# sunnyHelen/JPerceiver

Measured on AMD Instinct MI355X. Metric: train images/sec (full train step, synthetic 3-frame batches), higher is better.
Workload: dtype f32

## Files before the change

### jperceiver_amd/csrc/conv_pack.hip

```cpp
#include "conv_pack.h"
#include "igemm_p9.h"
#include "igemm_p9s.h"
#include "scale.h"
#include <algorithm>

namespace {

struct JpPackJob {
    const float* w;
    float* wp;
    long total, begin;
    int mode, p[6];
};
static_assert(sizeof(JpPackJob) == 64, "JpPackJob layout");
__host__ __device__ inline int jp_cdiv_d(int a, int b) { return (a + b - 1) / b; }

__device__ __forceinline__ float pack_slot_sum(const float* wc, int pl) {
    const int a = pl >> 3, b = (pl >> 2) & 1, r = (pl >> 1) & 1, sx = pl & 1;
    const int y0 = a ? (r ? 2 : 0) : (r ? 1 : 0), y1 = a ? (r ? 2 : 1) : (r ? 2 : 0);
    const int x0 = b ? (sx ? 2 : 0) : (sx ? 1 : 0), x1 = b ? (sx ? 2 : 1) : (sx ? 2 : 0);
    float v = 0.f;
    for (int dy = y0; dy <= y1; ++dy)
        for (int dx = x0; dx <= x1; ++dx) v += wc[dy * 3 + dx];
    return v;
}

__device__ __forceinline__ float pack_elem(int mode, const float* __restrict__ w, long i, const int* p, float sc = 1.f) {
    switch (mode) {
        case PACK_TAP: {
            const int Cout = p[0], Cin = p[1], KHW = p[2], Cp = p[3], for_dgrad = p[4];
            const int rows = for_dgrad ? Cin : Cout, red = for_dgrad ? Cout : Cin;
            const int c = (int)(i % Cp);
            const long t = i / Cp;
            const int r = (int)(t % rows), tap = (int)(t / rows);
            if (c >= red) return 0.f;
            const int co = for_dgrad ? c : r, ci = for_dgrad ? r : c;
            return w[((size_t)co * Cin + ci) * KHW + tap];
        }
        case PACK_ROWMAJOR: {
            const int Cin = p[1], KHW = p[2], CP = p[3], Kp = p[4];
            const int k = (int)(i % Kp), m = (int)(i / Kp);
            const int tap = k / CP, c = k - tap * CP;
            return (tap < KHW && c < Cin) ? w[((size_t)m * Cin + c) * KHW + tap] : 0.f;
        }
        case PACK_SEG: {
            const int Cout = p[0], Cin = p[1], c_off = p[2], C = p[3], Cp = p[4], up = p[5];
            const int c = (int)(i % Cp);
            const long t = i / Cp;
            const int co = (int)(t % Cout), pl = (int)(t / Cout);
            if (c >= C) return 0.f;
            const float* wc = w + ((size_t)co * Cin + c_off + c) * 9;
            return up ? pack_slot_sum(wc, pl) : wc[pl];
        }
        case PACK_UP_DGRAD: {
            const int Cout = p[0], Cin = p[1], c_off = p[2], Cx = p[3], Cp = p[4];
            const int co = (int)(i % Cp);
            const long t = i / Cp;
            const int c = (int)(t % Cx), pl = (int)(t / Cx);
            if (co >= Cout) return 0.f;
            return pack_slot_sum(w + ((size_t)co * Cin + c_off + c) * 9, pl);
        }
        case PACK_FRAG: {
            const int Cout = p[0], Cin = p[1], for_dgrad = p[2], BMT = p[3], KHW = p[4];
            const int rows = for_dgrad ? Cin : Cout, red = for_dgrad ? Cout : Cin;
            const long per_tile = ((long)((red + 31) / 32) * KHW * 4 + P9_QAHEAD + 1) * 8 * BMT;
            const int mt = (int)(i / per_tile);
            long t = i - (long)mt * per_tile;
            const int j = (int)(t & 3); t >>= 2;
            const int m = mt * BMT + (int)(t % BMT);
            t /= BMT;
            const int par = (int)(t & 1); t >>= 1;
            const long step = t * 4 + j;
            const int s_ = (int)(step & 15);
            const long tc = step >> 4;
            const int tap = (int)(tc % KHW);
            const int c = (int)(tc / KHW) * 32 + 2 * s_ + par;
            if (m >= rows || c >= red) return 0.f;
            const int co = for_dgrad ? c : m, ci = for_dgrad ? m : c;
            return w[((size_t)co * Cin + ci) * KHW + tap];
        }
        case PACK_SPLIT: {
            const int Cout = p[0], Cin = p[1], for_dgrad = p[2], BMT = p[3], KHW = p[4], KGS = p[5];
            const int rows = for_dgrad ? Cin : Cout, red = for_dgrad ? Cout : Cin;
            const long nsteps = (long)(red / (16 * KGS)) * KHW * KGS;
            const long per_tile = (nsteps + P9S_AHEAD) * (JP_NS * 8) * BMT;
            const int mt = (int)(i / per_tile);
            long t = i - (long)mt * per_tile;
            const int w4 = (int)(t & 3); t >>= 2;
            const int m = mt * BMT + (int)(t % BMT);
            t /= BMT;
            const int khalf = (int)(t & 1); t >>= 1;
            const int sp = (int)(t % JP_NS);
            const long U = t / JP_NS;
            if (U >= nsteps || m >= rows) return 0.f;
            const int stage = (int)(U / (KHW * KGS)), u = (int)(U % (KHW * KGS));
            const int tap = u / KGS, kg = u % KGS;
            const int c = stage * 16 * KGS + kg * 16 + khalf * 8 + 2 * w4;
            float v[2];
#pragma unroll
            for (int k = 0; k < 2; ++k) {
                const int cc = c + k;
                const int co = for_dgrad ? cc : m, ci = for_dgrad ? m : cc;
                v[k] = cc < red ? w[((size_t)co * Cin + ci) * KHW + tap] : 0.f;
            }
            unsigned sq[3];
            jp_split_ns(v[0], v[1], sc, sq);
            return __uint_as_float(sp == 0 ? sq[0] : (sp == 1 ? sq[1] : sq[2]));
        }
        case PACK_SPLIT7: {
            const int Cout = p[0], Cin = p[1];
            const int w4 = (int)(i & 3), m = (int)((i >> 2) & 63), khalf = (int)((i >> 8) & 1);
            const long t = i >> 9;
            const int sp = (int)(t % JP_NS);
            const long U = t / JP_NS;
            const int c = (int)(U >> 2), ky = 2 * (int)(U & 3) + khalf;
            float v[2];
#pragma unroll
            for (int k = 0; k < 2; ++k) {
                const int kx = 2 * w4 + k;
                v[k] = (c < Cin && m < Cout && ky < 7 && kx < 7) ? w[(((size_t)m * Cin + c) * 7 + ky) * 7 + kx] : 0.f;
            }
            unsigned sq[3];
            jp_split_ns(v[0], v[1], sc, sq);
            return __uint_as_float(sp == 0 ? sq[0] : (sp == 1 ? sq[1] : sq[2]));
        }
        case PACK_SPLITUPD: {
            const int Cout = p[0], Cin = p[1], c_off = p[2], Cx = p[3];
            const long nsteps = (long)((Cout + 31) / 32 * 2) * 16;
            const long per_tile = (nsteps + P9S_AHEAD) * (JP_NS * 1024);
            const int mt = (int)(i / per_tile);
            long t = i - (long)mt * per_tile;
            const int w4 = (int)(t & 3); t >>= 2;
            const int c = mt * 128 + (int)(t & 127); t >>= 7;
            const int khalf = (int)(t & 1); t >>= 1;
            const int sp = (int)(t % JP_NS);
            const long U = t / JP_NS;
            if (U >= nsteps || c >= Cx) return 0.f;
            const int stage = (int)(U >> 4), q = (int)(U & 15);
            const int co = stage * 16 + khalf * 8 + 2 * w4;
            float v[2];
#pragma unroll
            for (int k = 0; k < 2; ++k)
                v[k] = co + k < Cout ? pack_slot_sum(w + ((size_t)(co + k) * Cin + c_off + c) * 9, q) : 0.f;
            unsigned sq[3];
            jp_split_ns(v[0], v[1], sc, sq);
            return __uint_as_float(sp == 0 ? sq[0] : (sp == 1 ? sq[1] : sq[2]));
        }
        case PACK_SPLITSEG: {
            const int Cout = p[0], Cin = p[1], c_off = p[2], C = p[3], up = p[4];
            const int T = up ? 4 : 9, MT = Cout / 128;
            const long tile = (long)((C + 15) / 16) * T * (JP_NS * 1024);
            const int cm = (int)(i / tile);
            if (cm >= (up ? 4 : 1) * MT) return 0.f;
            long t = i - (long)cm * tile;
            const int cls = cm / MT, mt = cm - cls * MT;
            const int w4 = (int)(t & 3); t >>= 2;
            const int row = (int)(t & 127); t >>= 7;
            const int khalf = (int)(t & 1); t >>= 1;
            const int sp = (int)(t % JP_NS);
            const int U = (int)(t / JP_NS);
            const int stage = U / T, tap = U - stage * T;
            const int c = stage * 16 + khalf * 8 + 2 * w4, co = mt * 128 + row;
            float v[2];
#pragma unroll
            for (int k = 0; k < 2; ++k) {
                const float* wc = w + ((size_t)co * Cin + c_off + c + k) * 9;
                v[k] = (c + k < C && co < Cout) ? (up ? pack_slot_sum(wc, cls * 4 + tap) : wc[tap]) : 0.f;
            }
            unsigned sq[3];
            jp_split_ns(v[0], v[1], sc, sq);
            return __uint_as_float(sp == 0 ? sq[0] : (sp == 1 ? sq[1] : sq[2]));
        }
        case PACK_FRAGSEG: {
            const int Cout = p[0], Cin = p[1], c_off = p[2], C = p[3], KP = p[4], up = p[5];
            const int T = up ? 4 : 9, MT = Cout / 128;
            const long tile = (long)((C + 2 * KP - 1) / (2 * KP)) * T * KP / 4 * 1024;
            const int cm = (int)(i / tile);
            long t = i - (long)cm * tile;
            const int cls = cm / MT, mt = cm - cls * MT;
            const int j = (int)(t & 3); t >>= 2;
            const int row = (int)(t & 127); t >>= 7;
            const int par = (int)(t & 1); t >>= 1;
            const long step = t * 4 + j;
            const int stage = (int)(step / (T * KP)), rem = (int)(step - (long)stage * (T * KP));
            const int tap = rem / KP, s_ = rem - tap * KP;
            const int c = stage * 2 * KP + 2 * s_ + par, co = mt * 128 + row;
            if (c >= C || co >= Cout) return 0.f;
            const float* wc = w + ((size_t)co * Cin + c_off + c) * 9;
            return up ? pack_slot_sum(wc, cls * 4 + tap) : wc[tap];
        }
        default: {
            const int Cout = p[0], Cin = p[1], c_off = p[2];
            const int t = (int)(i % 9), co = (int)((i / 9) % Cout), c = (int)(i / (9 * (long)Cout));
            return w[((size_t)co * Cin + c_off + c) * 9 + 8 - t];
        }
    }
}

__device__ __forceinline__ int pack_hdr(int mode) { return (mode == PACK_SPLIT || mode == PACK_SPLITUPD || mode == PACK_SPLIT7) ? JP_PACK_HDR : 0; }
__device__ __forceinline__ float pack_scale_of(const JpPackJob& j) {
    if (!JP_PACK_HDR) return 1.f;
    if (j.mode == PACK_SPLIT || j.mode == PACK_SPLITUPD || j.mode == PACK_SPLIT7) return j.wp[0];
    if (j.mode == PACK_SPLITSEG) return *(j.wp - j.p[5]);
    return 1.f;
}
constexpr int PSL = 32;
__device__ __forceinline__ float* pack_scale_hdr(const JpPackJob& j, long* n) {
    const bool seg = j.mode == PACK_SPLITSEG && j.p[2] == 0;
    const bool upd = j.mode == PACK_SPLITUPD;
    const bool s7 = j.mode == PACK_SPLIT7;
    if (!JP_PACK_HDR || !(j.mode == PACK_SPLIT || seg || upd || s7)) return nullptr;
    *n = (long)j.p[0] * j.p[1] * ((seg || upd) ? 9 : (s7 ? 49 : j.p[4]));
    return seg ? j.wp - j.p[5] : j.wp;
}
__device__ __forceinline__ void pack_scale_zero(const JpPackJob& j) {
    long n;
    float* hdr = pack_scale_hdr(j, &n);
    if (hdr && threadIdx.x == 0) reinterpret_cast<unsigned*>(hdr)[2] = 0u;
}
__device__ __forceinline__ void pack_scale_reduce(const JpPackJob& j, int slice) {
    long n;
    float* hdr = pack_scale_hdr(j, &n);
    if (!hdr) return;
    const long per = (n + PSL - 1) / PSL, beg = slice * per, end = min(n, beg + per);
    unsigned m = 0;
    for (long i = beg + threadIdx.x; i < end; i += 256) m = max(m, jp_amag(__float_as_uint(j.w[i])));
#pragma unroll
    for (int o = 32; o > 0; o >>= 1) m = max(m, (unsigned)__shfl_xor((int)m, o, 64));
    if ((threadIdx.x & 63) == 0 && m) atomicMax(reinterpret_cast<unsigned*>(hdr) + 2, m);
}
__device__ __forceinline__ void pack_scale_finish(const JpPackJob& j) {
    long n;
    float* hdr = pack_scale_hdr(j, &n);
    if (!hdr || threadIdx.x) return;
    const int k = jp_scale_exp(hdr[2] * ((j.mode == PACK_SPLITSEG || j.mode == PACK_SPLITUPD) ? 4.f : 1.f));
    hdr[0] = jp_exp2i(k);
    hdr[1] = jp_exp2i(-k);
    hdr[2] = hdr[3] = 0.f;
}
__global__ __launch_bounds__(64) void pack_scale_zero_one_kernel(JpPackJob job) { pack_scale_zero(job); }
__global__ __launch_bounds__(256) void pack_scale_reduce_one_kernel(JpPackJob job) { pack_scale_reduce(job, blockIdx.x); }
__global__ __launch_bounds__(64) void pack_scale_finish_one_kernel(JpPackJob job) { pack_scale_finish(job); }
__global__ __launch_bounds__(64) void pack_scale_zero_kernel(const JpPackJob* __restrict__ jobs, int njobs) {
    const int q = blockIdx.x * 64 + threadIdx.x;
    if (q < njobs) { long n; float* hdr = pack_scale_hdr(jobs[q], &n); if (hdr) reinterpret_cast<unsigned*>(hdr)[2] = 0u; }
}
__global__ __launch_bounds__(256) void pack_scale_reduce_kernel(const JpPackJob* __restrict__ jobs, int njobs) {
    pack_scale_reduce(jobs[blockIdx.y], blockIdx.x);
}
__global__ __launch_bounds__(64) void pack_scale_finish_kernel(const JpPackJob* __restrict__ jobs, int njobs) {
    const int q = blockIdx.x * 64 + threadIdx.x;
    if (q < njobs) {
        long n;
        float* hdr = pack_scale_hdr(jobs[q], &n);
        if (hdr) {
            const int k = jp_scale_exp(hdr[2] * ((jobs[q].mode == PACK_SPLITSEG || jobs[q].mode == PACK_SPLITUPD) ? 4.f : 1.f));
            hdr[0] = jp_exp2i(k);
            hdr[1] = jp_exp2i(-k);
            hdr[2] = hdr[3] = 0.f;
        }
    }
}

__global__ __launch_bounds__(256) void pack_one_kernel(JpPackJob job) {
    const int hdr = pack_hdr(job.mode);
    const float sc = pack_scale_of(job);
    for (long i = (long)blockIdx.x * 256 + threadIdx.x; i < job.total - hdr; i += (long)gridDim.x * 256)
        job.wp[hdr + i] = pack_elem(job.mode, job.w, i, job.p, sc);
}

__global__ __launch_bounds__(256) void pack_replay_kernel(const JpPackJob* __restrict__ jobs, int njobs, long total) {
    const long groups = (total + 3) >> 2;
    for (long g4 = (long)blockIdx.x * 256 + threadIdx.x; g4 < groups; g4 += (long)gridDim.x * 256) {
        const long g = g4 << 2;
        int lo = 0, hi = njobs - 1;
        while (lo < hi) {
            const int mid = (lo + hi + 1) >> 1;
            if (jobs[mid].begin <= g) lo = mid; else hi = mid - 1;
        }
        const JpPackJob& j = jobs[lo];
        const long i = g - j.begin;
        if (i >= j.total) continue;
        if (j.mode == PACK_SPLIT || j.mode == PACK_SPLITSEG) continue;
        if (j.mode == PACK_FRAG && i + 4 <= j.total) {
            const int* p = j.p;
            const int Cout = p[0], Cin = p[1], for_dgrad = p[2], BMT = p[3], KHW = p[4];
            const int rows = for_dgrad ? Cin : Cout, red = for_dgrad ? Cout : Cin;
            const long per_tile = ((long)((red + 31) / 32) * KHW * 4 + P9_QAHEAD + 1) * 8 * BMT;
            const int mt = (int)(i / per_tile);
            long t = (i - (long)mt * per_tile) >> 2;
            const int m = mt * BMT + (int)(t % BMT);
            t /= BMT;
            const int par = (int)(t & 1); t >>= 1;
            const long step = t * 4;
            const int s0 = (int)(step & 15);
            const long tc = step >> 4;
            const int tap = (int)(tc % KHW), c0 = (int)(tc / KHW) * 32 + 2 * s0 + par;
            float4 v = make_float4(0.f, 0.f, 0.f, 0.f);
            if (m < rows) {
                const size_t cs = for_dgrad ? (size_t)Cin * KHW : (size_t)KHW;
                const float* wb = j.w + (for_dgrad ? (size_t)m * KHW : (size_t)m * Cin * KHW) + tap;
                if (c0 < red) v.x = wb[(size_t)c0 * cs];
                if (c0 + 2 < red) v.y = wb[(size_t)(c0 + 2) * cs];
                if (c0 + 4 < red) v.z = wb[(size_t)(c0 + 4) * cs];
                if (c0 + 6 < red) v.w = wb[(size_t)(c0 + 6) * cs];
            }
            *reinterpret_cast<float4*>(j.wp + i) = v;
        } else {
            const int hdr = pack_hdr(j.mode);
            const float sc = hdr ? pack_scale_of(j) : 1.f;
#pragma unroll
            for (int k = 0; k < 4; ++k)
                if (i + k >= hdr && i + k < j.total) j.wp[i + k] = pack_elem(j.mode, j.w, i + k - hdr, j.p, sc);
        }
    }
}

__device__ __forceinline__ int split_job_items(const JpPackJob& j) {
    const int* p = j.p;
    if (j.mode == PACK_SPLIT) {
        const int rows = p[2] ? p[1] : p[0], red = p[2] ? p[0] : p[1];
        return jp_cdiv_d(rows, p[3]) * (red / (16 * p[5])) * (p[3] / 64);
    }
    if (j.mode == PACK_SPLITSEG) return (p[0] / 128) * ((p[3] + 15) / 16) * 2;
    return 0;
}
__global__ __launch_bounds__(256) void pack_split_replay_kernel(const JpPackJob* __restrict__ jobs, int njobs) {
    __shared__ float tile[64 * 16 * 9 + 64];
    constexpr int MAXJ = 2048;
    __shared__ int pre[MAXJ + 1];
    const int t = threadIdx.x;
    for (int q = t; q < njobs && q < MAXJ; q += 256) pre[q + 1] = split_job_items(jobs[q]);
    if (t == 0) pre[0] = 0;
    __syncthreads();
    if (t == 0)
        for (int q = 1; q <= njobs && q <= MAXJ; ++q) pre[q] += pre[q - 1];
    __syncthreads();
    const int nj = min(njobs, MAXJ), total_items = pre[nj];
    for (int item = blockIdx.x; item < total_items; item += gridDim.x) {
        __syncthreads();
        int lo = 0, hi = nj - 1;
        while (lo < hi) {
            const int mid = (lo + hi + 1) >> 1;
            if (pre[mid] <= item) lo = mid; else hi = mid - 1;
        }
        const int jj = lo, loc = item - pre[lo];
        const JpPackJob& j = jobs[jj];
        const int* p = j.p;
        unsigned* out = reinterpret_cast<unsigned*>(j.wp) + pack_hdr(j.mode);
        if (j.mode == PACK_SPLIT) {
            const float wsc = JP_PACK_HDR ? j.wp[0] : 1.f;
            const int Cout = p[0], Cin = p[1], for_dgrad = p[2], BMT = p[3], KHW = p[4], KGS = p[5];
            const int rows = for_dgrad ? Cin : Cout, red = for_dgrad ? Cout : Cin;
            const int CS = 16 * KGS, nst = red / CS, rch = BMT / 64;
            const int rc = loc % rch, stage = (loc / rch) % nst, mt = loc / (rch * nst);
            const int m0 = mt * BMT + rc * 64, c0 = stage * CS;
            const int RUN = CS * KHW;
            if (!for_dgrad) {
                for (int e = t; e < 64 * RUN; e += 256) {
                    const int r = e / RUN, o = e - r * RUN;
                    tile[e] = (m0 + r < rows) ? j.w[((size_t)(m0 + r) * Cin + c0) * KHW + o] : 0.f;
                }
            } else {
                const int RUNd = 64 * KHW;
                for (int e = t; e < CS * RUNd; e += 256) {
                    const int c = e / RUNd, o = e - c * RUNd;
                    tile[e] = (m0 + o / KHW < rows) ? j.w[((size_t)(c0 + c) * Cin + m0) * KHW + o] : 0.f;
                }
            }
            __syncthreads();
            const long nsteps = (long)nst * KHW * KGS;
            const long per_tile = (nsteps + P9S_AHEAD) * (JP_NS * 8) * BMT;
            const int trip = KHW * KGS * 2 * 64;
            for (int e = t; e < trip; e += 256) {
                const int r = e & 63, kh = (e >> 6) & 1, u = e >> 7;
                const int tap = u / KGS, kg = u - tap * KGS;
                jp_u32x4 w0, w1, w2;
#pragma unroll
                for (int k = 0; k < 4; ++k) {
                    const int c = kg * 16 + kh * 8 + 2 * k;
                    const float a = for_dgrad ? tile[(c * 64 + r) * KHW + tap] : tile[(r * CS + c) * KHW + tap];
                    const float b = for_dgrad ? tile[((c + 1) * 64 + r) * KHW + tap] : tile[(r * CS + c + 1) * KHW + tap];
                    unsigned sq[3];
                    jp_split_ns(a, b, wsc, sq);
                    w0[k] = sq[0]; w1[k] = sq[1]; w2[k] = sq[2];
                }
                const long U = (long)stage * KHW * KGS + u;
                unsigned* q = out + (long)mt * per_tile + ((U * JP_NS) * 2 + kh) * (long)BMT * 4 + (long)(rc * 64 + r) * 4;
                *reinterpret_cast<jp_u32x4*>(q) = w0;
                *reinterpret_cast<jp_u32x4*>(q + 2L * BMT * 4) = w1;
                if (JP_NS == 3) *reinterpret_cast<jp_u32x4*>(q + 4L * BMT * 4) = w2;
            }
        } else {
            const int Cout = p[0], Cin = p[1], c_off = p[2], C = p[3], up = p[4];
            const int T = up ? 4 : 9, MT = Cout / 128, nst = (C + 15) / 16;
            const int rc = loc & 1, stage = (loc >> 1) % nst, mt = (loc >> 1) / nst;
            const int m0 = mt * 128 + rc * 64, c0 = stage * 16;
            for (int e = t; e < 64 * 144; e += 256) {
                const int r = e / 144, o = e - r * 144, c = o / 9;
                tile[e] = (c0 + c < C && m0 + r < Cout) ? j.w[((size_t)(m0 + r) * Cin + c_off + c0) * 9 + o] : 0.f;
            }
            __syncthreads();
            const long tl = (long)nst * T * (JP_NS * 1024);
            const int ncls = up ? 4 : 1, trip = ncls * T * 2 * 64;
            const float wsc = pack_scale_of(j);
            for (int e = t; e < trip; e += 256) {
                const int r = e & 63, kh = (e >> 6) & 1, ct = e >> 7, tap = ct % T, cls = ct / T;
                jp_u32x4 w0, w1, w2;
#pragma unroll
                for (int k = 0; k < 4; ++k) {
                    const int c = kh * 8 + 2 * k;
                    const float* wa = tile + (r * 16 + c) * 9;
                    const float a = up ? pack_slot_sum(wa, cls * 4 + tap) : wa[tap];
                    const float b = up ? pack_slot_sum(wa + 9, cls * 4 + tap) : wa[9 + tap];
                    unsigned sq[3];
                    jp_split_ns(a, b, wsc, sq);
                    w0[k] = sq[0]; w1[k] = sq[1]; w2[k] = sq[2];
                }
                const long U = (long)stage * T + tap;
                unsigned* q = out + (long)(cls * MT + mt) * tl + ((U * JP_NS) * 2 + kh) * 512L + (long)(rc * 64 + r) * 4;
                *reinterpret_cast<jp_u32x4*>(q) = w0;
                *reinterpret_cast<jp_u32x4*>(q + 1024) = w1;
                if (JP_NS == 3) *reinterpret_cast<jp_u32x4*>(q + 2048) = w2;
            }
        }
    }
}

thread_local JpPackJob* g_pack_rec = nullptr;
thread_local int g_pack_rec_n = 0, g_pack_rec_cap = 0;

}

void do_pack(int mode, const float* w, float* wp, long total, int p0, int p1, int p2, int p3, int p4, int p5, hipStream_t st) {
    JpPackJob j{w, wp, total, 0, mode, {p0, p1, p2, p3, p4, p5}};
    if (g_pack_rec) {
        if (g_pack_rec_n < g_pack_rec_cap) g_pack_rec[g_pack_rec_n] = j;
        ++g_pack_rec_n;
    }
    if (JP_PACK_HDR && (mode == PACK_SPLIT || mode == PACK_SPLITUPD || mode == PACK_SPLIT7 || (mode == PACK_SPLITSEG && p2 == 0))) {
        hipLaunchKernelGGL(pack_scale_zero_one_kernel, dim3(1), dim3(64), 0, st, j);
        hipLaunchKernelGGL(pack_scale_reduce_one_kernel, dim3(PSL), dim3(256), 0, st, j);
        hipLaunchKernelGGL(pack_scale_finish_one_kernel, dim3(1), dim3(64), 0, st, j);
    }
    hipLaunchKernelGGL(pack_one_kernel, dim3((int)std::min<long>((total + 255) / 256, 4096)), dim3(256), 0, st, j);
}

void pack_weights(const float* w, float* wp, int Cout, int Cin, int KHW, int Cp, int for_dgrad, hipStream_t st) {
    do_pack(PACK_TAP, w, wp, (long)KHW * (for_dgrad ? Cin : Cout) * Cp, Cout, Cin, KHW, Cp, for_dgrad, 0, st);
}

extern "C" int jp_pack_job_bytes(void) { return (int)sizeof(JpPackJob); }

extern "C" int jp_pack_record_begin(void* host_jobs, int max_jobs) {
    JP_CHECK_ARG(host_jobs && max_jobs > 0 && !g_pack_rec, "pack_record_begin: bad args or a recording is already open");
    g_pack_rec = (JpPackJob*)host_jobs;
    g_pack_rec_n = 0;
    g_pack_rec_cap = max_jobs;
    return JP_OK;
}

extern "C" int jp_pack_record_end(void) {
    g_pack_rec = nullptr;
    return g_pack_rec_n;
}

extern "C" int jp_pack_mode_is_split(int mode) { return (mode == PACK_SPLIT || mode == PACK_SPLITSEG) ? 1 : 0; }
extern "C" int jp_pack_replay(const void* jobs, int njobs, long total_elems, long generic_elems, void* stream) {
    JP_CHECK_ARG(jobs && njobs > 0 && total_elems > 0, "pack_replay: bad args");
    const long gen = (generic_elems > 0 && generic_elems < total_elems) ? generic_elems : total_elems;
    if (JP_PACK_HDR)
    {
        hipLaunchKernelGGL(pack_scale_zero_kernel, dim3((njobs + 63) / 64), dim3(64), 0, (hipStream_t)stream, (const JpPackJob*)jobs, njobs);
        hipLaunchKernelGGL(pack_scale_reduce_kernel, dim3(PSL, njobs), dim3(256), 0, (hipStream_t)stream, (const JpPackJob*)jobs, njobs);
        hipLaunchKernelGGL(pack_scale_finish_kernel, dim3((njobs + 63) / 64), dim3(64), 0, (hipStream_t)stream, (const JpPackJob*)jobs, njobs);
    }
    hipLaunchKernelGGL(pack_replay_kernel, dim3((int)std::min<long>((gen + 4095) / 4096, 16384)), dim3(256), 0,
                       (hipStream_t)stream, (const JpPackJob*)jobs, njobs, gen);
    for (int off = 0; off < njobs; off += 2048)
        hipLaunchKernelGGL(pack_split_replay_kernel, dim3(4096), dim3(256), 0, (hipStream_t)stream, (const JpPackJob*)jobs + off,
                           std::min(2048, njobs - off));
    JP_LAUNCH_CHECK();
}
```

Measured before the change: 126.7.

## Add fast weight-pack replay path with vectorized reduce, walk scheduling, pipelined split pack

Adds an env-gated fast path, on by default, for weight-pack replay. The scale reduction now reads float4 vectors. The generic replay kernel gives each block a contiguous range, walks jobs linearly instead of binary-searching per element, and gets a vectorized PACK_TAP case. A new persistent split-pack kernel stages coalesced tiles through registers and shared memory, prefetching the next item while the current one is stored. This targets per-step weight repacking overhead, at the cost of more code and register pressure.

After: 123.9. -2.2%, worse.

```diff
diff --git a/jperceiver_amd/csrc/conv_pack.hip b/jperceiver_amd/csrc/conv_pack.hip
--- a/jperceiver_amd/csrc/conv_pack.hip
+++ b/jperceiver_amd/csrc/conv_pack.hip
@@ -248,6 +248,30 @@
 __global__ __launch_bounds__(256) void pack_scale_reduce_kernel(const JpPackJob* __restrict__ jobs, int njobs) {
     pack_scale_reduce(jobs[blockIdx.y], blockIdx.x);
 }
+__global__ __launch_bounds__(256) void pack_scale_reduce4_kernel(const JpPackJob* __restrict__ jobs, int njobs) {
+    const JpPackJob& j = jobs[blockIdx.y];
+    long n;
+    float* hdr = pack_scale_hdr(j, &n);
+    if (!hdr) return;
+    const int t = threadIdx.x, slice = blockIdx.x;
+    const long head = min(n, (long)((16 - ((uintptr_t)j.w & 15)) & 15) >> 2);
+    const float4* w4 = reinterpret_cast<const float4*>(j.w + head);
+    const long n4 = (n - head) >> 2, per = (n4 + PSL - 1) / PSL, beg = slice * per, end = min(n4, beg + per);
+    unsigned m = 0;
+    for (long i = beg + t; i < end; i += 256) {
+        const float4 v = w4[i];
+        m = max(max(m, jp_amag(__float_as_uint(v.x))), jp_amag(__float_as_uint(v.y)));
+        m = max(max(m, jp_amag(__float_as_uint(v.z))), jp_amag(__float_as_uint(v.w)));
+    }
+    if (slice == 0) {
+        if (t < head) m = max(m, jp_amag(__float_as_uint(j.w[t])));
+        const long tail = head + (n4 << 2);
+        if (tail + t < n) m = max(m, jp_amag(__float_as_uint(j.w[tail + t])));
+    }
+#pragma unroll
+    for (int o = 32; o > 0; o >>= 1) m = max(m, (unsigned)__shfl_xor((int)m, o, 64));
+    if ((t & 63) == 0 && m) atomicMax(reinterpret_cast<unsigned*>(hdr) + 2, m);
+}
 __global__ __launch_bounds__(64) void pack_scale_finish_kernel(const JpPackJob* __restrict__ jobs, int njobs) {
     const int q = blockIdx.x * 64 + threadIdx.x;
     if (q < njobs) {
@@ -269,6 +293,57 @@
         job.wp[hdr + i] = pack_elem(job.mode, job.w, i, job.p, sc);
 }
 
+template <bool FAST>
+__device__ __forceinline__ void pack_replay_group(const JpPackJob& j, long i) {
+    if (i >= j.total) return;
+    if (j.mode == PACK_SPLIT || j.mode == PACK_SPLITSEG) return;
+    if (j.mode == PACK_FRAG && i + 4 <= j.total) {
+        const int* p = j.p;
+        const int Cout = p[0], Cin = p[1], for_dgrad = p[2], BMT = p[3], KHW = p[4];
+        const int rows = for_dgrad ? Cin : Cout, red = for_dgrad ? Cout : Cin;
+        const long per_tile = ((long)((red + 31) / 32) * KHW * 4 + P9_QAHEAD + 1) * 8 * BMT;
+        const int mt = (int)(i / per_tile);
+        long t = (i - (long)mt * per_tile) >> 2;
+        const int m = mt * BMT + (int)(t % BMT);
+        t /= BMT;
+        const int par = (int)(t & 1); t >>= 1;
+        const long step = t * 4;
+        const int s0 = (int)(step & 15);
+        const long tc = step >> 4;
+        const int tap = (int)(tc % KHW), c0 = (int)(tc / KHW) * 32 + 2 * s0 + par;
+        float4 v = make_float4(0.f, 0.f, 0.f, 0.f);
+        if (m < rows) {
+            const size_t cs = for_dgrad ? (size_t)Cin * KHW : (size_t)KHW;
+            const float* wb = j.w + (for_dgrad ? (size_t)m * KHW : (size_t)m * Cin * KHW) + tap;
+            if (c0 < red) v.x = wb[(size_t)c0 * cs];
+            if (c0 + 2 < red) v.y = wb[(size_t)(c0 + 2) * cs];
+            if (c0 + 4 < red) v.z = wb[(size_t)(c0 + 4) * cs];
+            if (c0 + 6 < red) v.w = wb[(size_t)(c0 + 6) * cs];
+        }
+        *reinterpret_cast<float4*>(j.wp + i) = v;
+    } else if (FAST && j.mode == PACK_TAP && (j.p[3] & 3) == 0 && i + 4 <= j.total && j.total < (1L << 31) &&
+               ((uintptr_t)(j.wp + i) & 15) == 0) {
+        const int* p = j.p;
+        const unsigned Cout = p[0], Cin = p[1], KHW = p[2], Cp = p[3];
+        const bool for_dgrad = p[4] != 0;
+        const unsigned rows = for_dgrad ? Cin : Cout, red = for_dgrad ? Cout : Cin;
+        const unsigned iu = (unsigned)i, t = iu / Cp, c = iu - t * Cp, tap = t / rows, r = t - tap * rows;
+        const size_t cs = for_dgrad ? (size_t)Cin * KHW : (size_t)KHW;
+        const float* wb = j.w + (for_dgrad ? (size_t)r * KHW : (size_t)r * Cin * KHW) + tap;
+        float4 v = make_float4(0.f, 0.f, 0.f, 0.f);
+        if (c < red) v.x = wb[(size_t)c * cs];
+        if (c + 1 < red) v.y = wb[(size_t)(c + 1) * cs];
+        if (c + 2 < red) v.z = wb[(size_t)(c + 2) * cs];
+        if (c + 3 < red) v.w = wb[(size_t)(c + 3) * cs];
+        *reinterpret_cast<float4*>(j.wp + i) = v;
+    } else {
+        const int hdr = pack_hdr(j.mode);
+        const float sc = hdr ? pack_scale_of(j) : 1.f;
+#pragma unroll
+        for (int k = 0; k < 4; ++k)
+            if (i + k >= hdr && i + k < j.total) j.wp[i + k] = pack_elem(j.mode, j.w, i + k - hdr, j.p, sc);
+    }
+}
 __global__ __launch_bounds__(256) void pack_replay_kernel(const JpPackJob* __restrict__ jobs, int njobs, long total) {
     const long groups = (total + 3) >> 2;
     for (long g4 = (long)blockIdx.x * 256 + threadIdx.x; g4 < groups; g4 += (long)gridDim.x * 256) {
@@ -278,41 +353,31 @@
             const int mid = (lo + hi + 1) >> 1;
             if (jobs[mid].begin <= g) lo = mid; else hi = mid - 1;
         }
-        const JpPackJob& j = jobs[lo];
-        const long i = g - j.begin;
-        if (i >= j.total) continue;
-        if (j.mode == PACK_SPLIT || j.mode == PACK_SPLITSEG) continue;
-        if (j.mode == PACK_FRAG && i + 4 <= j.total) {
-            const int* p = j.p;
-            const int Cout = p[0], Cin = p[1], for_dgrad = p[2], BMT = p[3], KHW = p[4];
-            const int rows = for_dgrad ? Cin : Cout, red = for_dgrad ? Cout : Cin;
-            const long per_tile = ((long)((red + 31) / 32) * KHW * 4 + P9_QAHEAD + 1) * 8 * BMT;
-            const int mt = (int)(i / per_tile);
-            long t = (i - (long)mt * per_tile) >> 2;
-            const int m = mt * BMT + (int)(t % BMT);
-            t /= BMT;
-            const int par = (int)(t & 1); t >>= 1;
-            const long step = t * 4;
-            const int s0 = (int)(step & 15);
-            const long tc = step >> 4;
-            const int tap = (int)(tc % KHW), c0 = (int)(tc / KHW) * 32 + 2 * s0 + par;
-            float4 v = make_float4(0.f, 0.f, 0.f, 0.f);
-            if (m < rows) {
-                const size_t cs = for_dgrad ? (size_t)Cin * KHW : (size_t)KHW;
-                const float* wb = j.w + (for_dgrad ? (size_t)m * KHW : (size_t)m * Cin * KHW) + tap;
-                if (c0 < red) v.x = wb[(size_t)c0 * cs];
-                if (c0 + 2 < red) v.y = wb[(size_t)(c0 + 2) * cs];
-                if (c0 + 4 < red) v.z = wb[(size_t)(c0 + 4) * cs];
-                if (c0 + 6 < red) v.w = wb[(size_t)(c0 + 6) * cs];
-            }
-            *reinterpret_cast<float4*>(j.wp + i) = v;
-        } else {
-            const int hdr = pack_hdr(j.mode);
-            const float sc = hdr ? pack_scale_of(j) : 1.f;
-#pragma unroll
-            for (int k = 0; k < 4; ++k)
-                if (i + k >= hdr && i + k < j.total) j.wp[i + k] = pack_elem(j.mode, j.w, i + k - hdr, j.p, sc);
-        }
+        pack_replay_group<false>(jobs[lo], g - jobs[lo].begin);
+    }
+}
+__global__ __launch_bounds__(256) void pack_replay_walk_kernel(const JpPackJob* __restrict__ jobs, int njobs, long total) {
+    const long groups = (total + 3) >> 2;
+    const long per = ((groups + gridDim.x - 1) / gridDim.x + 255) & ~255L;
+    const long gb = (long)blockIdx.x * per, ge = min(groups, gb + per);
+    if (gb >= ge) return;
+    int lo = 0, hi = njobs - 1;
+    while (lo < hi) {
+        const int mid = (lo + hi + 1) >> 1;
+        if (jobs[mid].begin <= (gb << 2)) lo = mid; else hi = mid - 1;
+    }
+    long next = lo + 1 < njobs ? jobs[lo + 1].begin : total;
+    JpPackJob cur = jobs[lo];
+    for (long g4 = gb + threadIdx.x; g4 < ge; g4 += 256) {
+        const long g = g4 << 2;
+        if (next <= g) {
+            while (lo + 1 < njobs && next <= g) {
+                ++lo;
+                next = lo + 1 < njobs ? jobs[lo + 1].begin : total;
+            }
+            cur = jobs[lo];
+        }
+        pack_replay_group<true>(cur, g - cur.begin);
     }
 }
 
@@ -427,6 +492,234 @@
     }
 }
 
+typedef float psf_f4 __attribute__((ext_vector_type(4)));
+constexpr int PSF_MAXJ = 512;
+constexpr int PSF_SLOTS = 10;
+struct PsfItem {
+    const JpPackJob* j;
+    const float* w;
+    size_t stride;
+    int nr, rl, ls;
+    int vruns, vlen;
+    int al, sm, nch;
+    int loc;
+};
+__device__ __forceinline__ PsfItem psf_decode(const JpPackJob* jq, int loc) {
+    PsfItem it;
+    const JpPackJob& j = *jq;
+    const int* p = j.p;
+    it.j = jq;
+    it.loc = loc;
+    size_t base;
+    if (j.mode == PACK_SPLIT) {
+        const int Cout = p[0], Cin = p[1], for_dgrad = p[2], BMT = p[3], KHW = p[4], KGS = p[5];
+        const int rows = for_dgrad ? Cin : Cout, red = for_dgrad ? Cout : Cin;
+        const int CS = 16 * KGS, nst = red / CS, rch = BMT / 64;
+        const int rc = loc % rch, stage = (loc / rch) % nst, mt = loc / (rch * nst);
+        const int m0 = mt * BMT + rc * 64, c0 = stage * CS;
+        const int left = min(64, max(0, rows - m0));
+        it.stride = (size_t)Cin * KHW;
+        if (!for_dgrad) {
+            it.nr = 64; it.rl = CS * KHW; it.vruns = left; it.vlen = it.rl;
+            base = ((size_t)m0 * Cin + c0) * KHW;
+        } else {
+            it.nr = CS; it.rl = 64 * KHW; it.vruns = CS; it.vlen = left * KHW;
+            base = ((size_t)c0 * Cin + m0) * KHW;
+        }
+    } else {
+        const int Cout = p[0], Cin = p[1], c_off = p[2], C = p[3];
+        const int nst = (C + 15) / 16;
+        const int rc = loc & 1, stage = (loc >> 1) % nst, mt = (loc >> 1) / nst;
+        const int m0 = mt * 128 + rc * 64, c0 = stage * 16;
+        it.stride = (size_t)Cin * 9;
+        it.nr = 64; it.rl = 144; it.vruns = min(64, max(0, Cout - m0)); it.vlen = min(16, C - c0) * 9;
+        base = ((size_t)m0 * Cin + c_off + c0) * 9;
+    }
+    it.w = j.w + base;
+    it.ls = it.rl | 1;
+    it.al = (int)(((uintptr_t)it.w >> 2) & 3);
+    it.sm = (int)(it.stride & 3);
+    it.nch = it.rl / 4 + ((it.al | it.sm) ? 1 : 0);
+    return it;
+}
+#define PSF_FOR_CHUNKS(it)                                                                                 \
+    const int nchunks_ = it.nr * it.nch, dk_ = 256 / it.nch, dj_ = 256 - dk_ * it.nch;                     \
+    int k = (int)threadIdx.x / it.nch, jc_ = (int)threadIdx.x - k * it.nch;                                \
+    _Pragma("unroll") for (int s = 0; s < PSF_SLOTS; ++s, k += dk_ + (jc_ + dj_ >= it.nch), jc_ += dj_ - (jc_ + dj_ >= it.nch ? it.nch : 0)) \
+        if (s * 256 + (int)threadIdx.x < nchunks_)
+__device__ __forceinline__ void psf_load(const PsfItem& it, psf_f4 (&rg)[PSF_SLOTS]) {
+    PSF_FOR_CHUNKS(it) {
+        const int o0 = 4 * jc_ - ((it.al + k * it.sm) & 3);
+        const int vl = k < it.vruns ? it.vlen : 0;
+        const float* src = it.w + ((long)k * (long)it.stride + o0);
+        if (o0 >= 0 && o0 + 4 <= vl) {
+            rg[s] = *reinterpret_cast<const psf_f4*>(src);
+        } else {
+            rg[s].x = (o0 >= 0 && o0 < vl) ? src[0] : 0.f;
+            rg[s].y = (o0 + 1 >= 0 && o0 + 1 < vl) ? src[1] : 0.f;
+            rg[s].z = (o0 + 2 >= 0 && o0 + 2 < vl) ? src[2] : 0.f;
+            rg[s].w = (o0 + 3 >= 0 && o0 + 3 < vl) ? src[3] : 0.f;
+        }
+    }
+}
+__device__ __forceinline__ void psf_stage(const PsfItem& it, const psf_f4 (&rg)[PSF_SLOTS], float* tile) {
+    const int rot = ((int)threadIdx.x >> 3) & 3;
+    PSF_FOR_CHUNKS(it) {
+        const int o0 = 4 * jc_ - ((it.al + k * it.sm) & 3);
+        float* d = tile + k * it.ls + o0;
+#pragma unroll
+        for (int e = 0; e < 4; ++e) {
+            const int c = (e + rot) & 3;
+            const float v = c == 0 ? rg[s].x : (c == 1 ? rg[s].y : (c == 2 ? rg[s].z : rg[s].w));
+            if (o0 + c >= 0 && o0 + c < it.rl) d[c] = v;
+        }
+    }
+}
+#undef PSF_FOR_CHUNKS
+__device__ __forceinline__ void psf_split_store(const PsfItem& it, const float* tile) {
+    const JpPackJob& j = *it.j;
+    const int* p = j.p;
+    const int t = threadIdx.x, loc = it.loc, LS = it.ls;
+    unsigned* out = reinterpret_cast<unsigned*>(j.wp) + pack_hdr(j.mode);
+    if (j.mode == PACK_SPLIT) {
+        const float wsc = JP_PACK_HDR ? j.wp[0] : 1.f;
+        const int Cout = p[0], Cin = p[1], for_dgrad = p[2], BMT = p[3], KHW = p[4], KGS = p[5];
+        const int red = for_dgrad ? Cout : Cin;
+        const int CS = 16 * KGS, nst = red / CS, rch = BMT / 64;
+        const int rc = loc % rch, stage = (loc / rch) % nst, mt = loc / (rch * nst);
+        const long nsteps = (long)nst * KHW * KGS;
+        const long per_tile = (nsteps + P9S_AHEAD) * (JP_NS * 8) * BMT;
+        const int trip = KHW * KGS * 2 * 64;
+        for (int e = t; e < trip; e += 256) {
+            const int r = e & 63, kh = (e >> 6) & 1, u = e >> 7;
+            const int tap = KGS == 1 ? u : (KGS == 2 ? u >> 1 : u / KGS), kg = u - tap * KGS;
+            const float* src = for_dgrad ? tile + (kg * 16 + kh * 8) * LS + r * KHW + tap : tile + r * LS + (kg * 16 + kh * 8) * KHW + tap;
+            const int cst = for_dgrad ? LS : KHW;
+            jp_u32x4 w0, w1, w2;
+#pragma unroll
+            for (int k = 0; k < 4; ++k) {
+                unsigned sq[3];
+                jp_split_ns(src[2 * k * cst], src[(2 * k + 1) * cst], wsc, sq);
+                w0[k] = sq[0]; w1[k] = sq[1]; w2[k] = sq[2];
+            }
+            const long U = (long)stage * KHW * KGS + u;
+            unsigned* q = out + (long)mt * per_tile + ((U * JP_NS) * 2 + kh) * (long)BMT * 4 + (long)(rc * 64 + r) * 4;
+            *reinterpret_cast<jp_u32x4*>(q) = w0;
+            *reinterpret_cast<jp_u32x4*>(q + 2L * BMT * 4) = w1;
+            if (JP_NS == 3) *reinterpret_cast<jp_u32x4*>(q + 4L * BMT * 4) = w2;
+        }
+        if (stage == nst - 1)
+            for (int e = t; e < P9S_AHEAD * JP_NS * 2 * 64; e += 256) {
+                const int r = e & 63, x = e >> 6;
+                unsigned* q = out + (long)mt * per_tile + (nsteps * JP_NS * 2 + x) * (long)BMT * 4 + (long)(rc * 64 + r) * 4;
+                *reinterpret_cast<jp_u32x4*>(q) = jp_u32x4{0u, 0u, 0u, 0u};
+            }
+    } else {
+        const int Cout = p[0], C = p[3], up = p[4];
+        const int T = up ? 4 : 9, MT = Cout / 128, nst = (C + 15) / 16;
+        const int rc = loc & 1, stage = (loc >> 1) % nst, mt = (loc >> 1) / nst;
+        const long tl = (long)nst * T * (JP_NS * 1024);
+        const int ncls = up ? 4 : 1, trip = ncls * T * 2 * 64;
+        const float wsc = pack_scale_of(j);
+        for (int e = t; e < trip; e += 256) {
+            const int r = e & 63, kh = (e >> 6) & 1, ct = e >> 7;
+            const int cls = up ? ct >> 2 : 0, tap = up ? ct & 3 : ct;
+            jp_u32x4 w0, w1, w2;
+#pragma unroll
+            for (int k = 0; k < 4; ++k) {
+                const float* wa = tile + r * LS + (kh * 8 + 2 * k) * 9;
+                const float a = up ? pack_slot_sum(wa, cls * 4 + tap) : wa[tap];
+                const float b = up ? pack_slot_sum(wa + 9, cls * 4 + tap) : wa[9 + tap];
+                unsigned sq[3];
+                jp_split_ns(a, b, wsc, sq);
+                w0[k] = sq[0]; w1[k] = sq[1]; w2[k] = sq[2];
+            }
+            const long U = (long)stage * T + tap;
+            unsigned* q = out + (long)(cls * MT + mt) * tl + ((U * JP_NS) * 2 + kh) * 512L + (long)(rc * 64 + r) * 4;
+            *reinterpret_cast<jp_u32x4*>(q) = w0;
+            *reinterpret_cast<jp_u32x4*>(q + 1024) = w1;
+            if (JP_NS == 3) *reinterpret_cast<jp_u32x4*>(q + 2048) = w2;
+        }
+    }
+}
+__global__ __launch_bounds__(256) void pack_split_fast_kernel(const JpPackJob* __restrict__ jobs, int njobs) {
+    __shared__ float tile[64 * 145];
+    constexpr int MAXJ = PSF_MAXJ, PER = MAXJ / 256;
+    __shared__ int pre[MAXJ + 1];
+    __shared__ int wsum[4];
+    const int t = threadIdx.x, nj = min(njobs, MAXJ);
+    {
+        int cnt[PER], sum = 0;
+#pragma unroll
+        for (int q = 0; q < PER; ++q) {
+            cnt[q] = PER * t + q < nj ? split_job_items(jobs[PER * t + q]) : 0;
+            sum += cnt[q];
+        }
+        int inc = sum;
+#pragma unroll
+        for (int o = 1; o < 64; o <<= 1) {
+            const int v = __shfl_up(inc, o, 64);
+            if ((t & 63) >= o) inc += v;
+        }
+        if ((t & 63) == 63) wsum[t >> 6] = inc;
+        __syncthreads();
+        int run = inc - sum;
+        for (int wv = 0; wv < (t >> 6); ++wv) run += wsum[wv];
+        if (t == 0) pre[0] = 0;
+#pragma unroll
+        for (int q = 0; q < PER; ++q) {
+            run += cnt[q];
+            if (PER * t + q < nj) pre[PER * t + q + 1] = run;
+        }
+        __syncthreads();
+    }
+    const int total_items = pre[nj];
+    int item = blockIdx.x;
+    if (item >= total_items) return;
+    int jj;
+    {
+        int lo = 0, hi = nj - 1;
+        while (lo < hi) {
+            const int mid = (lo + hi + 1) >> 1;
+            if (pre[mid] <= item) lo = mid; else hi = mid - 1;
+        }
+        jj = lo;
+    }
+    psf_f4 rg[PSF_SLOTS];
+    PsfItem cur = psf_decode(jobs + jj, item - pre[jj]);
+    psf_load(cur, rg);
+    while (true) {
+        psf_stage(cur, rg, tile);
+        __syncthreads();
+        const int nxt = item + gridDim.x;
+        PsfItem nx = cur;
+        if (nxt < total_items) {
+            while (pre[jj + 1] <= nxt) ++jj;
+            nx = psf_decode(jobs + jj, nxt - pre[jj]);
+            psf_load(nx, rg);
+        }
+        psf_split_store(cur, tile);
+        if (nxt >= total_items) break;
+        __syncthreads();
+        cur = nx;
+        item = nxt;
+    }
+}
+
+bool pack_fast() {
+    static const bool on = [] { const char* e = getenv("JP_PACK_FAST"); return !(e && e[0] == '0'); }();
+    return on;
+}
+int pack_split_fast_grid() {
+    static const int g = [] {
+        int dev = 0, cus = 0;
+        if (hipGetDevice(&dev) != hipSuccess || hipDeviceGetAttribute(&cus, hipDeviceAttributeMultiprocessorCount, dev) != hipSuccess || cus <= 0)
+            cus = 256;
+        return 4 * cus;
+    }();
+    return g;
+}
+
 thread_local JpPackJob* g_pack_rec = nullptr;
 thread_local int g_pack_rec_n = 0, g_pack_rec_cap = 0;
 
@@ -472,13 +765,16 @@
     if (JP_PACK_HDR)
     {
         hipLaunchKernelGGL(pack_scale_zero_kernel, dim3((njobs + 63) / 64), dim3(64), 0, (hipStream_t)stream, (const JpPackJob*)jobs, njobs);
-        hipLaunchKernelGGL(pack_scale_reduce_kernel, dim3(PSL, njobs), dim3(256), 0, (hipStream_t)stream, (const JpPackJob*)jobs, njobs);
+        hipLaunchKernelGGL(pack_fast() ? pack_scale_reduce4_kernel : pack_scale_reduce_kernel, dim3(PSL, njobs), dim3(256), 0, (hipStream_t)stream,
+                           (const JpPackJob*)jobs, njobs);
         hipLaunchKernelGGL(pack_scale_finish_kernel, dim3((njobs + 63) / 64), dim3(64), 0, (hipStream_t)stream, (const JpPackJob*)jobs, njobs);
     }
-    hipLaunchKernelGGL(pack_replay_kernel, dim3((int)std::min<long>((gen + 4095) / 4096, 16384)), dim3(256), 0,
+    const bool fast = pack_fast();
+    hipLaunchKernelGGL(fast ? pack_replay_walk_kernel : pack_replay_kernel, dim3((int)std::min<long>((gen + 4095) / 4096, 16384)), dim3(256), 0,
                        (hipStream_t)stream, (const JpPackJob*)jobs, njobs, gen);
-    for (int off = 0; off < njobs; off += 2048)
-        hipLaunchKernelGGL(pack_split_replay_kernel, dim3(4096), dim3(256), 0, (hipStream_t)stream, (const JpPackJob*)jobs + off,
-                           std::min(2048, njobs - off));
+    const int slice = fast ? PSF_MAXJ : 2048;
+    for (int off = 0; off < njobs; off += slice)
+        hipLaunchKernelGGL(fast ? pack_split_fast_kernel : pack_split_replay_kernel, dim3(fast ? pack_split_fast_grid() : 4096), dim3(256), 0,
+                           (hipStream_t)stream, (const JpPackJob*)jobs + off, std::min(slice, njobs - off));
     JP_LAUNCH_CHECK();
 }
```
